# JiawangBian/SC-SfMLearner-Release

Measured on AMD Instinct MI355X. Metric: train images/sec (+ warp-loss ms/step) KITTI 256x832 RN18, higher is better.
Workload: dtype f32; 1 GPU; configs[1]: kitti 256x832, batch 12/GPU, 2 refs (seq 3), ResNet18 DispNet + ResNet18 PoseNet, ssim+mask+auto-mask, zeros padding, 1 scale; global_batch=12, parallelism=1 GPU, memory_format=contiguous (NCHW)

## Files before the change

__graft_entry__.py:

```python
import os
import sys

ROOT = os.path.dirname(os.path.abspath(__file__))
PKG = os.path.join(ROOT, "sc-sfmlearner-release_amd")
for p in (ROOT, PKG):
    if p not in sys.path:
        sys.path.insert(0, p)


def build() -> None:
    from scsfm_hip import _lib, build as hip_build
    path = hip_build.build(force=False)
    lib = _lib.CLib(path)
    assert lib._dll.scsfm_abi_version() == _lib.ABI_VERSION
    nets_path = hip_build.build_nets(force=False)
    nets = _lib.CLib(nets_path, _lib.NETS_HEADER, _lib.NETS_ABI_VERSION, "scsfm_nets_")
    eval_path = hip_build.build_eval(force=False)
    ev = _lib.CLib(eval_path, _lib.EVAL_HEADER, _lib.EVAL_ABI_VERSION, "scsfm_eval_")
    odom_path = hip_build.build_odom(force=False)
    od = _lib.CLib(odom_path, _lib.ODOM_HEADER, _lib.ODOM_ABI_VERSION, "scsfm_odom_")
    enc_path = hip_build.build_enc(force=False)
    enc = _lib.CLib(enc_path, _lib.ENC_HEADER, _lib.ENC_ABI_VERSION, "scsfm_enc_")
    import inverse_warp
    import loss_functions
    import models
    from scsfm_hip import decoder, depth_eval, encoder, odometry
    from oracle import scsfm_oracle
    print(f"[build] {path}: {len(lib.decls)} entry points resolved")
    print(f"[build] {nets_path}: {len(nets.decls)} entry points resolved")
    print(f"[build] {eval_path}: {len(ev.decls)} entry points resolved")
    print(f"[build] {odom_path}: {len(od.decls)} entry points resolved")
    print(f"[build] {enc_path}: {len(enc.decls)} entry points resolved")


def smoke() -> None:
    import torch

    import loss_functions as LF
    from oracle import scsfm_oracle as O
    from scsfm_hip import _lib, synth

    assert torch.cuda.is_available(), "smoke() needs a HIP device"
    lib = _lib.get()
    assert lib.path.endswith("libscsfm_hip.so")
    dev = torch.device("cuda:0")
    d = synth.make_batch(2, 128, 416, n_ref=2, seed=0, depth="smooth")

    def leaves(device):
        mv = lambda t: t.to(device).clone().requires_grad_(True)
        return ([mv(t) for t in d["tgt_depth"]], [[mv(t) for t in r] for r in d["ref_depths"]],
                [mv(p) for p in d["poses"]], [mv(p) for p in d["poses_inv"]])

    td, rd, ps, pi = leaves(dev)
    tgt, refs, K = d["tgt_img"].to(dev), [r.to(dev) for r in d["ref_imgs"]], d["intrinsics"].to(dev)
    photo, geom = LF.compute_photo_and_geometry_loss(tgt, refs, K, td, rd, ps, pi, 1, 1, 1, 1, "zeros")
    smooth = LF.compute_smooth_loss(td, tgt, rd, refs)
    (photo + 0.1 * smooth + 0.5 * geom).backward()
    torch.cuda.synchronize()

    td_c, rd_c, ps_c, pi_c = leaves("cpu")
    photo_c, geom_c = O.photo_and_geometry_loss(d["tgt_img"], d["ref_imgs"], d["intrinsics"], td_c, rd_c, ps_c, pi_c,
                                                1, 1, 1, 1, "zeros")
    smooth_c = O.smooth_loss(td_c, d["tgt_img"], rd_c, d["ref_imgs"])
    (photo_c + 0.1 * smooth_c + 0.5 * geom_c).backward()
    for name, a, b in (("photo", photo, photo_c), ("geom", geom, geom_c), ("smooth", smooth, smooth_c)):
        err = abs(float(a) - float(b))
        print(f"[smoke] {name}: hip {float(a):.7f} oracle {float(b):.7f} |d| {err:.2e}")
        assert err <= 1e-5, name
    pairs = [("g_tgt_depth", td[0].grad, td_c[0].grad), ("g_ref0_depth", rd[0][0].grad, rd_c[0][0].grad),
             ("g_ref1_depth", rd[1][0].grad, rd_c[1][0].grad), ("g_pose0", ps[0].grad, ps_c[0].grad),
             ("g_pose_inv1", pi[1].grad, pi_c[1].grad)]
    for name, a, b in pairs:
        scale = float(b.abs().max())
        bad = ((a.cpu() - b).abs() > 0.01 * scale).double().mean().item()
        print(f"[smoke] {name}: scale {scale:.3e} share of entries off by >1% of scale {bad:.2e}")
        assert bad <= 2e-3, name
    print("[smoke] ok")


if __name__ == "__main__":
    build()
    if "--smoke" in sys.argv:
        smoke()
```

sc-sfmlearner-release_amd/models/resnet_encoder.py:

```python
from __future__ import absolute_import, division, print_function

import numpy as np
import torch
import torch.nn as nn


_encoder_ops = None


def _E():
    global _encoder_ops
    if _encoder_ops is None:
        from scsfm_hip import encoder
        _encoder_ops = encoder
    return _encoder_ops


def _fused_applies(x, *bns):
    return x.is_cuda and _E().applies(x, *bns)


def _bn_act(x, bn, act, identity=None):
    if _fused_applies(x, bn) and (identity is None or _fused_applies(identity)):
        return _E().bn_act(x, bn, identity, relu=act is not None)
    out = bn(x)
    if identity is not None:
        out = out + identity
    return out if act is None else act(out)


def _downsample(ds, x):
    return _bn_act(ds[0](x), ds[1], None)


def _conv3x3(cin, cout, stride=1):
    return nn.Conv2d(cin, cout, kernel_size=3, stride=stride, padding=1, bias=False)


class BasicBlock(nn.Module):
    expansion = 1

    def __init__(self, inplanes, planes, stride=1, downsample=None):
        super().__init__()
        self.conv1 = _conv3x3(inplanes, planes, stride)
        self.bn1 = nn.BatchNorm2d(planes)
        self.relu = nn.ReLU(inplace=True)
        self.conv2 = _conv3x3(planes, planes)
        self.bn2 = nn.BatchNorm2d(planes)
        self.downsample = downsample

    def forward(self, x):
        identity = x if self.downsample is None else _downsample(self.downsample, x)
        out = _bn_act(self.conv1(x), self.bn1, self.relu)
        return _bn_act(self.conv2(out), self.bn2, self.relu, identity)

    def forward_reference(self, x):
        identity = x if self.downsample is None else self.downsample(x)
        out = self.relu(self.bn1(self.conv1(x)))
        out = self.bn2(self.conv2(out))
        return self.relu(out + identity)


class Bottleneck(nn.Module):
    expansion = 4

    def __init__(self, inplanes, planes, stride=1, downsample=None):
        super().__init__()
        self.conv1 = nn.Conv2d(inplanes, planes, kernel_size=1, bias=False)
        self.bn1 = nn.BatchNorm2d(planes)
        self.conv2 = _conv3x3(planes, planes, stride)
        self.bn2 = nn.BatchNorm2d(planes)
        self.conv3 = nn.Conv2d(planes, planes * 4, kernel_size=1, bias=False)
        self.bn3 = nn.BatchNorm2d(planes * 4)
        self.relu = nn.ReLU(inplace=True)
        self.downsample = downsample

    def forward(self, x):
        identity = x if self.downsample is None else _downsample(self.downsample, x)
        out = _bn_act(self.conv1(x), self.bn1, self.relu)
        out = _bn_act(self.conv2(out), self.bn2, self.relu)
        return _bn_act(self.conv3(out), self.bn3, self.relu, identity)

    def forward_reference(self, x):
        identity = x if self.downsample is None else self.downsample(x)
        out = self.relu(self.bn1(self.conv1(x)))
        out = self.relu(self.bn2(self.conv2(out)))
        out = self.bn3(self.conv3(out))
        return self.relu(out + identity)


class ResNet(nn.Module):

    def __init__(self, block, layers, num_classes=1000, num_input_images=1):
        super().__init__()
        self.inplanes = 64
        self.conv1 = nn.Conv2d(num_input_images * 3, 64, kernel_size=7, stride=2, padding=3, bias=False)
        self.bn1 = nn.BatchNorm2d(64)
        self.relu = nn.ReLU(inplace=True)
        self.maxpool = nn.MaxPool2d(kernel_size=3, stride=2, padding=1)
        self.layer1 = self._make_layer(block, 64, layers[0])
        self.layer2 = self._make_layer(block, 128, layers[1], stride=2)
        self.layer3 = self._make_layer(block, 256, layers[2], stride=2)
        self.layer4 = self._make_layer(block, 512, layers[3], stride=2)
        self.avgpool = nn.AdaptiveAvgPool2d((1, 1))
        self.fc = nn.Linear(512 * block.expansion, num_classes)
        for m in self.modules():
            if isinstance(m, nn.Conv2d):
                nn.init.kaiming_normal_(m.weight, mode='fan_out', nonlinearity='relu')
            elif isinstance(m, nn.BatchNorm2d):
                nn.init.constant_(m.weight, 1)
                nn.init.constant_(m.bias, 0)

    def _make_layer(self, block, planes, blocks, stride=1):
        downsample = None
        if stride != 1 or self.inplanes != planes * block.expansion:
            downsample = nn.Sequential(
                nn.Conv2d(self.inplanes, planes * block.expansion, kernel_size=1, stride=stride, bias=False),
                nn.BatchNorm2d(planes * block.expansion))
        layers = [block(self.inplanes, planes, stride, downsample)]
        self.inplanes = planes * block.expansion
        layers += [block(self.inplanes, planes) for _ in range(1, blocks)]
        return nn.Sequential(*layers)


_CFG = {18: (BasicBlock, [2, 2, 2, 2]), 50: (Bottleneck, [3, 4, 6, 3])}


def imagenet_weights_path(num_layers):
    import os
    root = os.environ.get("SCSFM_IMAGENET_WEIGHTS")
    if not root:
        return None
    path = os.path.join(root, "resnet{}.pth".format(num_layers))
    return path if os.path.exists(path) else None


class ResnetEncoder(nn.Module):

    def __init__(self, num_layers, pretrained, num_input_images=1):
        super().__init__()
        if num_layers not in _CFG:
            raise ValueError("{} is not a valid number of resnet layers".format(num_layers))
        block, layers = _CFG[num_layers]
        self.num_ch_enc = np.array([64, 64, 128, 256, 512])
        if num_layers > 34:
            self.num_ch_enc[1:] *= 4
        self.encoder = ResNet(block, layers, num_input_images=num_input_images)
        if pretrained:
            path = imagenet_weights_path(num_layers)
            if path is None:
                raise RuntimeError("ImageNet-pretrained weights are not reachable offline: set SCSFM_IMAGENET_WEIGHTS "
                                   "to a directory holding resnet{}.pth, or use --with-pretrain 0".format(num_layers))
            loaded = torch.load(path, map_location="cpu")
            loaded['conv1.weight'] = torch.cat([loaded['conv1.weight']] * num_input_images, 1) / num_input_images
            self.encoder.load_state_dict(loaded)
        for p in self.encoder.fc.parameters():
            p.requires_grad_(False)

    def forward(self, input_image):
        e = self.encoder
        f0 = _bn_act(e.conv1(input_image), e.bn1, e.relu)
        f1 = e.layer1(self._maxpool(f0))
        f2 = e.layer2(f1)
        f3 = e.layer3(f2)
        f4 = e.layer4(f3)
        self.features = [f0, f1, f2, f3, f4]
        return self.features

    def _maxpool(self, f0):
        e = self.encoder
        if f0.is_cuda and e.training and _E().pool_applies(f0):
            return _E().max_pool(f0)
        return e.maxpool(f0)

    def forward_reference(self, input_image):
        e = self.encoder
        f0 = e.relu(e.bn1(e.conv1(input_image)))
        feats, x = [f0], e.maxpool(f0)
        for layer in (e.layer1, e.layer2, e.layer3, e.layer4):
            for block in layer:
                x = block.forward_reference(x)
            feats.append(x)
        return feats
```

sc-sfmlearner-release_amd/scsfm_hip/_lib.py:

```python
from __future__ import annotations

import ctypes
import os
import re
import threading

import torch

HERE = os.path.dirname(os.path.abspath(__file__))
HEADER = os.path.join(os.path.dirname(os.path.dirname(HERE)), "include", "scsfm_hip.h")
LIB_PATH = os.environ.get("SCSFM_HIP_LIB") or os.path.join(HERE, "libscsfm_hip.so")

ABI_VERSION = 9

_CTYPES = {"int": ctypes.c_int, "unsigned": ctypes.c_uint, "size_t": ctypes.c_size_t, "double": ctypes.c_double}
_DECL = re.compile(r"^(int|size_t)\s+(scsfm_\w+)\s*\(([^)]*)\)\s*;", re.M | re.S)


def parse_header(path=HEADER):
    text = open(path).read()
    text = re.sub(r"/\*.*?\*/", "", text, flags=re.S)
    out = {}
    for ret, name, args in _DECL.findall(text):
        argtypes = []
        args = " ".join(args.split())
        if args and args != "void":
            for a in args.split(","):
                a = a.strip()
                if "*" in a:
                    argtypes.append(ctypes.c_void_p)
                else:
                    argtypes.append(_CTYPES[a.split()[0]])
        out[name] = (_CTYPES[ret], argtypes)
    return out


class ScsfmError(RuntimeError):
    pass


class CLib:

    def __init__(self, path, header=HEADER, abi=ABI_VERSION, prefix="scsfm_"):
        self.path = path
        self._dll = ctypes.CDLL(path)
        self.decls = parse_header(header)
        self._fn = {}
        self._prefix = prefix
        for name, (ret, argtypes) in self.decls.items():
            try:
                fn = getattr(self._dll, name)
            except AttributeError as e:
                raise ScsfmError(f"{path} does not export {name} (declared in {header})") from e
            fn.restype = ret
            fn.argtypes = argtypes
            self._fn[name] = fn
        if self._fn[prefix + "abi_version"]() != abi:
            raise ScsfmError(f"{path}: ABI version mismatch")

    def source_id(self):
        buf = ctypes.create_string_buffer(64)
        self._fn[self._prefix + "source_id"](buf, 64)
        return buf.value.decode()

    def call(self, name, *args):
        rc = self._fn[name](*args)
        if rc != 0:
            kind = "rejected argument" if rc == -1 else "hipError_t"
            raise ScsfmError(f"{name} failed with status {rc} ({kind})")

    def size(self, name, *args):
        return int(self._fn[name](*args))


_lock = threading.Lock()
_lib = None


def get() -> CLib:
    global _lib
    if _lib is None:
        with _lock:
            if _lib is None:
                from . import build as _build
                own = "SCSFM_HIP_LIB" not in os.environ
                if own and _build.is_stale():
                    have = _build.binary_source_id(LIB_PATH)
                    try:
                        _build.build()
                    except Exception as e:
                        what = f"was built from other sources ({have}) than the tree's ({_build.source_id()})" if have \
                            else "is missing (or carries no source id)"
                        raise ScsfmError(f"{LIB_PATH} {what} and cannot be built here: {e}") from e
                lib = CLib(LIB_PATH)
                if own and lib.source_id() != _build.source_id():
                    raise ScsfmError(f"{LIB_PATH}: its source id {lib.source_id()} is not the tree's {_build.source_id()}")
                _lib = lib
    return _lib


NETS_HEADER = os.path.join(os.path.dirname(os.path.dirname(HERE)), "include", "scsfm_nets.h")
NETS_LIB_PATH = os.path.join(HERE, "libscsfm_nets.so")
NETS_ABI_VERSION = 1
_nets = None


def get_nets() -> CLib:
    global _nets
    if _nets is None:
        with _lock:
            if _nets is None:
                from . import build as _build
                if _build.nets_is_stale():
                    have = _build.binary_source_id(NETS_LIB_PATH)
                    try:
                        _build.build_nets()
                    except Exception as e:
                        raise ScsfmError(f"{NETS_LIB_PATH} is stale or missing ({have}) and cannot be built here: {e}") \
                            from e
                lib = CLib(NETS_LIB_PATH, NETS_HEADER, NETS_ABI_VERSION, "scsfm_nets_")
                if lib.source_id() != _build.nets_source_id():
                    raise ScsfmError(f"{NETS_LIB_PATH}: its source id {lib.source_id()} is not the tree's "
                                     f"{_build.nets_source_id()}")
                _nets = lib
    return _nets


EVAL_HEADER = os.path.join(os.path.dirname(os.path.dirname(HERE)), "include", "scsfm_eval.h")
EVAL_LIB_PATH = os.path.join(HERE, "libscsfm_eval.so")
EVAL_ABI_VERSION = 1
_eval = None


def get_eval() -> CLib:
    global _eval
    if _eval is None:
        with _lock:
            if _eval is None:
                from . import build as _build
                if _build.eval_is_stale():
                    have = _build.binary_source_id(EVAL_LIB_PATH)
                    try:
                        _build.build_eval()
                    except Exception as e:
                        raise ScsfmError(f"{EVAL_LIB_PATH} is stale or missing ({have}) and cannot be built here: {e}") \
                            from e
                lib = CLib(EVAL_LIB_PATH, EVAL_HEADER, EVAL_ABI_VERSION, "scsfm_eval_")
                if lib.source_id() != _build.eval_source_id():
                    raise ScsfmError(f"{EVAL_LIB_PATH}: its source id {lib.source_id()} is not the tree's "
                                     f"{_build.eval_source_id()}")
                _eval = lib
    return _eval


ODOM_HEADER = os.path.join(os.path.dirname(os.path.dirname(HERE)), "include", "scsfm_odom.h")
ODOM_LIB_PATH = os.path.join(HERE, "libscsfm_odom.so")
ODOM_ABI_VERSION = 1
_odom = None


def get_odom() -> CLib:
    global _odom
    if _odom is None:
        with _lock:
            if _odom is None:
                from . import build as _build
                if _build.odom_is_stale():
                    have = _build.binary_source_id(ODOM_LIB_PATH)
                    try:
                        _build.build_odom()
                    except Exception as e:
                        raise ScsfmError(f"{ODOM_LIB_PATH} is stale or missing ({have}) and cannot be built here: {e}") \
                            from e
                lib = CLib(ODOM_LIB_PATH, ODOM_HEADER, ODOM_ABI_VERSION, "scsfm_odom_")
                if lib.source_id() != _build.odom_source_id():
                    raise ScsfmError(f"{ODOM_LIB_PATH}: its source id {lib.source_id()} is not the tree's "
                                     f"{_build.odom_source_id()}")
                _odom = lib
    return _odom


ENC_HEADER = os.path.join(os.path.dirname(os.path.dirname(HERE)), "include", "scsfm_enc.h")
ENC_LIB_PATH = os.path.join(HERE, "libscsfm_enc.so")
ENC_ABI_VERSION = 1
_enc = None


def get_enc() -> CLib:
    global _enc
    if _enc is None:
        with _lock:
            if _enc is None:
                from . import build as _build
                if _build.enc_is_stale():
                    have = _build.binary_source_id(ENC_LIB_PATH)
                    try:
                        _build.build_enc()
                    except Exception as e:
                        raise ScsfmError(f"{ENC_LIB_PATH} is stale or missing ({have}) and cannot be built here: {e}") \
                            from e
                lib = CLib(ENC_LIB_PATH, ENC_HEADER, ENC_ABI_VERSION, "scsfm_enc_")
                if lib.source_id() != _build.enc_source_id():
                    raise ScsfmError(f"{ENC_LIB_PATH}: its source id {lib.source_id()} is not the tree's "
                                     f"{_build.enc_source_id()}")
                _enc = lib
    return _enc
```

sc-sfmlearner-release_amd/scsfm_hip/build.py:

```python
from __future__ import annotations

import contextlib
import fcntl
import glob
import hashlib
import os
import shutil
import subprocess
import sys
import tempfile

HERE = os.path.dirname(os.path.abspath(__file__))
CSRC = os.path.join(os.path.dirname(HERE), "csrc")
LIB = os.path.join(HERE, "libscsfm_hip.so")
LOCK = LIB + ".lock"
LOG = LIB + ".buildlog"
INCLUDE = os.path.join(os.path.dirname(os.path.dirname(HERE)), "include")
NETS_CSRC = os.path.join(os.path.dirname(HERE), "csrc_nets")
NETS_LIB = os.path.join(HERE, "libscsfm_nets.so")
EVAL_CSRC = os.path.join(os.path.dirname(HERE), "csrc_eval")
EVAL_LIB = os.path.join(HERE, "libscsfm_eval.so")
ODOM_CSRC = os.path.join(os.path.dirname(HERE), "csrc_odom")
ODOM_LIB = os.path.join(HERE, "libscsfm_odom.so")
ENC_CSRC = os.path.join(os.path.dirname(HERE), "csrc_enc")
ENC_LIB = os.path.join(HERE, "libscsfm_enc.so")
ARCH = "gfx950"
FLAGS = ["-O3", "-std=c++17", "-fPIC", "-shared", f"--offload-arch={ARCH}", "-munsafe-fp-atomics",
         "-fno-gpu-rdc", "-Wall", "-Wno-unused-function",
         "-fno-slp-vectorize"]
ID_MARKER = b"scsfm-source-id:"


def sources():
    return sorted(glob.glob(os.path.join(CSRC, "*.hip")))


def deps():
    return sources() + sorted(glob.glob(os.path.join(CSRC, "*.h"))) + \
        [os.path.join(INCLUDE, "scsfm_hip.h")]


def nets_sources():
    return sorted(glob.glob(os.path.join(NETS_CSRC, "*.hip")))


def nets_deps():
    return nets_sources() + sorted(glob.glob(os.path.join(NETS_CSRC, "*.h"))) + [os.path.join(INCLUDE, "scsfm_nets.h")]


def eval_sources():
    return sorted(glob.glob(os.path.join(EVAL_CSRC, "*.hip")))


def eval_deps():
    return eval_sources() + sorted(glob.glob(os.path.join(EVAL_CSRC, "*.h"))) + [os.path.join(INCLUDE, "scsfm_eval.h")]


def odom_sources():
    return sorted(glob.glob(os.path.join(ODOM_CSRC, "*.hip")))


def odom_deps():
    return odom_sources() + sorted(glob.glob(os.path.join(ODOM_CSRC, "*.h"))) + [os.path.join(INCLUDE, "scsfm_odom.h")]


def enc_sources():
    return sorted(glob.glob(os.path.join(ENC_CSRC, "*.hip")))


def enc_deps():
    return enc_sources() + sorted(glob.glob(os.path.join(ENC_CSRC, "*.h"))) + [os.path.join(INCLUDE, "scsfm_enc.h")]


def _hash(files, extra=()):
    h = hashlib.sha256()
    for path in files:
        h.update(os.path.basename(path).encode())
        h.update(open(path, "rb").read())
    h.update(" ".join(FLAGS).encode())
    if extra:
        h.update(b"\0extra:" + " ".join(extra).encode())
    return h.hexdigest()[:16]


def source_id(extra=()):
    files = deps()
    if any("SCSFM_WITH_MARCH" in e or "variants" in e for e in extra):
        vsrc = os.path.join(os.path.dirname(os.path.dirname(HERE)), "variants", "src")
        files = files + sorted(p for p in glob.glob(os.path.join(vsrc, "*")) if os.path.isfile(p))
    return _hash(files, extra)


def nets_source_id():
    return _hash(nets_deps())


def eval_source_id():
    return _hash(eval_deps())


def odom_source_id():
    return _hash(odom_deps())


def enc_source_id():
    return _hash(enc_deps())


def binary_source_id(path=LIB):
    try:
        blob = open(path, "rb").read()
    except OSError:
        return None
    i = blob.find(ID_MARKER)
    if i < 0:
        return None
    j = i + len(ID_MARKER)
    return blob[j:j + 16].decode("ascii", "replace")


def is_stale():
    return binary_source_id(LIB) != source_id()


def nets_is_stale():
    return binary_source_id(NETS_LIB) != nets_source_id()


def eval_is_stale():
    return binary_source_id(EVAL_LIB) != eval_source_id()


def odom_is_stale():
    return binary_source_id(ODOM_LIB) != odom_source_id()


def enc_is_stale():
    return binary_source_id(ENC_LIB) != enc_source_id()


@contextlib.contextmanager
def _build_lock(lock=None):
    fd = os.open(lock or LOCK, os.O_CREAT | os.O_RDWR, 0o644)
    try:
        fcntl.flock(fd, fcntl.LOCK_EX)
        yield
    finally:
        try:
            fcntl.flock(fd, fcntl.LOCK_UN)
        finally:
            os.close(fd)


def build(force=False, verbose=True, extra=()):
    extra = tuple(extra)
    return _build(LIB, source_id(extra), sources(), extra, force, verbose)


def build_nets(force=False, verbose=True):
    return _build(NETS_LIB, nets_source_id(), nets_sources(), ("-I", INCLUDE), force, verbose)


def build_eval(force=False, verbose=True):
    return _build(EVAL_LIB, eval_source_id(), eval_sources(), ("-I", INCLUDE), force, verbose)


def build_odom(force=False, verbose=True):
    return _build(ODOM_LIB, odom_source_id(), odom_sources(), ("-I", INCLUDE), force, verbose)


def build_enc(force=False, verbose=True):
    return _build(ENC_LIB, enc_source_id(), enc_sources(), ("-I", INCLUDE), force, verbose)


def _build(lib, want, srcs, extra, force, verbose):
    if not force and binary_source_id(lib) == want:
        return lib
    with _build_lock(lib + ".lock"):
        if not force and binary_source_id(lib) == want:
            return lib
        hipcc = shutil.which("hipcc") or "/opt/rocm/bin/hipcc"
        name = os.path.basename(lib)
        if not os.path.exists(hipcc):
            raise RuntimeError(f"hipcc not found: {name} cannot be built on this machine")
        fd, tmp = tempfile.mkstemp(prefix=name[:-len(".so")] + ".", suffix=f".{os.getpid()}.tmp", dir=HERE)
        os.close(fd)
        try:
            cmd = [hipcc, *FLAGS, f'-DSCSFM_SOURCE_ID="{want}"', *extra, "-o", tmp, *srcs]
            if verbose:
                print("[scsfm_hip.build]", " ".join(cmd), flush=True)
            subprocess.run(cmd, check=True)
            os.chmod(tmp, 0o755)
            os.replace(tmp, lib)
            with open(lib + ".buildlog", "a") as f:
                f.write(f"{want} {os.getpid()}\n")
        finally:
            if os.path.exists(tmp):
                os.unlink(tmp)
    return lib


if __name__ == "__main__":
    build(force="--force" in sys.argv)
    build_nets(force="--force" in sys.argv)
    build_eval(force="--force" in sys.argv)
    build_odom(force="--force" in sys.argv)
    build_enc(force="--force" in sys.argv)
    print(LIB)
    print(NETS_LIB)
    print(EVAL_LIB)
    print(ODOM_LIB)
    print(ENC_LIB)
```

sc-sfmlearner-release_amd/scsfm_hip/encoder.py:

```python
from __future__ import annotations

import torch
from torch.autograd.function import once_differentiable

from . import _lib
from .capi import _stream


def _plain(t):
    return t.is_cuda and t.dtype == torch.float32 and t.is_contiguous()


def applies(x, *bns):
    if not (torch.is_tensor(x) and x.dim() == 4 and _plain(x) and x.numel() < 2 ** 31 and
            x.shape[0] * x.shape[2] * x.shape[3] >= 2):
        return False
    for bn in bns:
        if not (bn.training and bn.affine and bn.track_running_stats and bn.momentum is not None):
            return False
        if not all(_plain(t) for t in (bn.weight, bn.bias, bn.running_mean, bn.running_var)):
            return False
        if not (bn.num_batches_tracked.is_cuda and bn.num_batches_tracked.dtype == torch.int64):
            return False
    return True


def pool_applies(x):
    return torch.is_tensor(x) and x.dim() == 4 and _plain(x) and 0 < x.numel() < 2 ** 31


def _workspace(lib, x):
    B, C, H, W = x.shape
    n = lib.size("scsfm_enc_bn_workspace_bytes", B, C, H, W)
    return torch.empty(n // 8, dtype=torch.float64, device=x.device), n


class _BnAct(torch.autograd.Function):
    @staticmethod
    def forward(ctx, x, identity, weight, bias, bn, mode):
        lib = _lib.get_enc()
        B, C, H, W = x.shape
        if identity is not None and (identity.shape != x.shape or not _plain(identity)):
            raise ValueError(f"bn_act: identity {tuple(identity.shape)} does not match x {tuple(x.shape)}")
        y = torch.empty_like(x)
        stat = torch.empty((3, C), dtype=torch.float32, device=x.device)
        ws, n = _workspace(lib, x)
        lib.call("scsfm_enc_bn_fwd_f32", B, C, H, W, mode, float(bn.eps), float(bn.momentum), x.data_ptr(),
                 0 if identity is None else identity.data_ptr(), weight.data_ptr(), bias.data_ptr(), y.data_ptr(),
                 stat.data_ptr(), bn.running_mean.data_ptr(), bn.running_var.data_ptr(),
                 bn.num_batches_tracked.data_ptr(), ws.data_ptr(), n, _stream(x))
        ctx.mode = mode
        ctx.save_for_backward(x, weight, bias, stat, *((y,) if mode == 2 else ()))
        return y

    @staticmethod
    @once_differentiable
    def backward(ctx, g):
        lib = _lib.get_enc()
        g = g.contiguous()
        x, weight, bias, stat = ctx.saved_tensors[:4]
        y = ctx.saved_tensors[4] if ctx.mode == 2 else None
        B, C, H, W = x.shape
        dx = torch.empty_like(x)
        d_id = torch.empty_like(x) if ctx.mode == 2 else None
        dgamma = torch.empty(C, dtype=torch.float32, device=x.device)
        dbeta = torch.empty(C, dtype=torch.float32, device=x.device)
        ws, n = _workspace(lib, x)
        lib.call("scsfm_enc_bn_bwd_f32", B, C, H, W, ctx.mode, g.data_ptr(), x.data_ptr(),
                 0 if y is None else y.data_ptr(), weight.data_ptr(), bias.data_ptr(), stat.data_ptr(), dx.data_ptr(),
                 0 if d_id is None else d_id.data_ptr(), dgamma.data_ptr(), dbeta.data_ptr(), ws.data_ptr(), n,
                 _stream(x))
        return dx, d_id, dgamma, dbeta, None, None


class _MaxPool(torch.autograd.Function):
    @staticmethod
    def forward(ctx, x):
        B, C, H, W = x.shape
        PH, PW = (H - 1) // 2 + 1, (W - 1) // 2 + 1
        out = torch.empty((B, C, PH, PW), dtype=x.dtype, device=x.device)
        arg = torch.empty((B, C, PH, PW), dtype=torch.uint8, device=x.device)
        _lib.get_enc().call("scsfm_enc_maxpool_fwd_f32", B, C, H, W, x.data_ptr(), out.data_ptr(), arg.data_ptr(),
                            _stream(x))
        ctx.save_for_backward(arg)
        ctx.shape = (B, C, H, W)
        return out

    @staticmethod
    @once_differentiable
    def backward(ctx, g):
        g = g.contiguous()
        (arg,) = ctx.saved_tensors
        B, C, H, W = ctx.shape
        dx = torch.empty((B, C, H, W), dtype=g.dtype, device=g.device)
        _lib.get_enc().call("scsfm_enc_maxpool_bwd_f32", B, C, H, W, g.data_ptr(), arg.data_ptr(), dx.data_ptr(),
                            _stream(g))
        return dx


def bn_act(x, bn, identity=None, relu=True):
    if not applies(x, bn):
        raise ValueError("scsfm_hip.encoder.bn_act: CUDA fp32 contiguous NCHW input and a training-mode affine "
                         f"BatchNorm2d with running statistics only (got {x.device} {x.dtype} {tuple(x.shape)})")
    if identity is not None and not relu:
        raise ValueError("bn_act: the residual form ends in a ReLU")
    mode = 2 if identity is not None else (1 if relu else 0)
    return _BnAct.apply(x, identity, bn.weight, bn.bias, bn, mode)


def max_pool(x):
    if not pool_applies(x):
        raise ValueError("scsfm_hip.encoder.max_pool: CUDA fp32 contiguous NCHW tensors only "
                         f"(got {x.device} {x.dtype} {tuple(x.shape)})")
    return _MaxPool.apply(x)
```

Before: 137.1 images/s.

## Fuse encoder stem BatchNorm, ReLU and max-pool into one HIP kernel pair

Adds a new HIP library that computes the stem BatchNorm+ReLU output and the 3x3/stride-2 max-pool in the same pass, writing f0, the pooled tensor and argmax indices together. The backward kernel routes pooled gradients through the argmax, adds the skip gradient from f0, and computes the BN gradient in one sweep. The aim is to avoid re-reading the full-resolution f0 activation for the separate pool forward and to avoid materialising a separate pool-backward gradient. The trade-off is a more complex kernel with halo handling across strips and a new library to build and validate.

```diff
diff --git a/__graft_entry__.py b/__graft_entry__.py
--- a/__graft_entry__.py
+++ b/__graft_entry__.py
@@ -21,6 +21,8 @@
     od = _lib.CLib(odom_path, _lib.ODOM_HEADER, _lib.ODOM_ABI_VERSION, "scsfm_odom_")
     enc_path = hip_build.build_enc(force=False)
     enc = _lib.CLib(enc_path, _lib.ENC_HEADER, _lib.ENC_ABI_VERSION, "scsfm_enc_")
+    stem_path = hip_build.build_stem(force=False)
+    stem = _lib.CLib(stem_path, _lib.STEM_HEADER, _lib.STEM_ABI_VERSION, "scsfm_stem_")
     import inverse_warp
     import loss_functions
     import models
@@ -31,6 +33,7 @@
     print(f"[build] {eval_path}: {len(ev.decls)} entry points resolved")
     print(f"[build] {odom_path}: {len(od.decls)} entry points resolved")
     print(f"[build] {enc_path}: {len(enc.decls)} entry points resolved")
+    print(f"[build] {stem_path}: {len(stem.decls)} entry points resolved")
 
 
 def smoke() -> None:
@@ -75,6 +78,15 @@
         bad = ((a.cpu() - b).abs() > 0.01 * scale).double().mean().item()
         print(f"[smoke] {name}: scale {scale:.3e} share of entries off by >1% of scale {bad:.2e}")
         assert bad <= 2e-3, name
+    import torch.nn as nn
+    from scsfm_hip import encoder as E
+    assert _lib.get_stem().path.endswith("libscsfm_stem.so")
+    xs = torch.randn(2, 4, 6, 8, device=dev)
+    bn_a, bn_b = nn.BatchNorm2d(4).to(dev).train(), nn.BatchNorm2d(4).to(dev).train()
+    f0, pooled = E.bn_act(xs, bn_a, pool=True)
+    f0_ref = E.bn_act(xs, bn_b)
+    assert torch.equal(f0, f0_ref) and torch.equal(pooled, E.max_pool(f0_ref))
+    print("[smoke] stem: fused BatchNorm / ReLU / max-pool equals the separate ops")
     print("[smoke] ok")
 
 
diff --git a/include/scsfm_stem.h b/include/scsfm_stem.h
--- /dev/null
+++ b/include/scsfm_stem.h
@@ -0,0 +1,27 @@
+#ifndef SCSFM_STEM_H_
+#define SCSFM_STEM_H_
+
+#include <stddef.h>
+
+#ifdef __cplusplus
+extern "C" {
+#endif
+
+int scsfm_stem_abi_version(void);
+int scsfm_stem_source_id(char* buf, size_t n);
+
+size_t scsfm_stem_workspace_bytes(int B, int C, int H, int W);
+
+int scsfm_stem_fwd_f32(int B, int C, int H, int W, double eps, double momentum, const float* x, const float* gamma,
+                       const float* beta, float* f0, float* out, unsigned char* arg, float* stat, float* running_mean,
+                       float* running_var, long long* num_batches_tracked, void* ws, size_t ws_bytes, void* stream);
+
+int scsfm_stem_bwd_f32(int B, int C, int H, int W, const float* g_pool, const float* g_f0, const unsigned char* arg,
+                       const float* x, const float* gamma, const float* beta, const float* stat, float* dx,
+                       float* dgamma, float* dbeta, void* ws, size_t ws_bytes, void* stream);
+
+#ifdef __cplusplus
+}
+#endif
+
+#endif
diff --git a/sc-sfmlearner-release_amd/csrc_stem/scsfm_stem.hip b/sc-sfmlearner-release_amd/csrc_stem/scsfm_stem.hip
--- /dev/null
+++ b/sc-sfmlearner-release_amd/csrc_stem/scsfm_stem.hip
@@ -0,0 +1,599 @@
+#include <hip/hip_runtime.h>
+
+#include "scsfm_stem.h"
+
+namespace scsfm_stem {
+
+constexpr int kWave = 64;
+constexpr int kThreads = 256;
+constexpr int kWaves = kThreads / kWave;
+constexpr int kMaxSplit = 64;
+constexpr int kMaxPart = 256;
+constexpr int kTargetBlocks = 2048;
+constexpr int kUnroll = 4;
+
+template <int V>
+struct Pack {
+  float v[V];
+};
+template <int V>
+__device__ inline Pack<V> load(const float* __restrict__ p);
+template <>
+__device__ inline Pack<1> load<1>(const float* __restrict__ p) {
+  return {{p[0]}};
+}
+template <>
+__device__ inline Pack<4> load<4>(const float* __restrict__ p) {
+  const float4 t = *reinterpret_cast<const float4*>(p);
+  return {{t.x, t.y, t.z, t.w}};
+}
+
+__device__ inline int imin(int a, int b) { return a < b ? a : b; }
+__device__ inline int imax(int a, int b) { return a > b ? a : b; }
+
+struct Geo {
+  int C, HW, per, units;
+};
+template <int V>
+__device__ inline int offset_of(const Geo& g, int c, int u) {
+  const int b = u / g.per;
+  return (b * g.C + c) * g.HW + (u - b * g.per) * V;
+}
+__device__ inline void range(const Geo& g, int& u0, int& u1) {
+  const long long S = gridDim.y, s = blockIdx.y;
+  u0 = (int)(g.units * s / S);
+  u1 = (int)(g.units * (s + 1) / S);
+}
+
+__device__ inline double wave_sum(double v) {
+#pragma unroll
+  for (int d = kWave / 2; d > 0; d >>= 1) v += __shfl_down(v, d);
+  return v;
+}
+
+__device__ inline void block_sum_to(double a, double b, double* __restrict__ dst) {
+  __shared__ double red[2 * kWaves];
+  a = wave_sum(a);
+  b = wave_sum(b);
+  const int lane = threadIdx.x & (kWave - 1), wave = threadIdx.x >> 6;
+  if (lane == 0) {
+    red[2 * wave] = a;
+    red[2 * wave + 1] = b;
+  }
+  __syncthreads();
+  if (threadIdx.x == 0) {
+    double ta = red[0], tb = red[1];
+#pragma unroll
+    for (int w = 1; w < kWaves; ++w) {
+      ta += red[2 * w];
+      tb += red[2 * w + 1];
+    }
+    dst[0] = ta;
+    dst[1] = tb;
+  }
+}
+
+__device__ inline void stat_totals(const double* __restrict__ part, int c, int S, double& a, double& b) {
+  const int lane = threadIdx.x & (kWave - 1);
+  const double* src = part + 2 * ((size_t)c * S + imin(lane, S - 1));
+  a = wave_sum(lane < S ? src[0] : 0.0);
+  b = wave_sum(lane < S ? src[1] : 0.0);
+}
+
+__device__ inline void part_totals(const double* __restrict__ part, int c, int G, double& a, double& b) {
+  const int lane = threadIdx.x & (kWave - 1);
+  double sa = 0.0, sb = 0.0;
+  for (int j = lane; j < G; j += kWave) {
+    const double* src = part + 2 * ((size_t)c * G + j);
+    sa += src[0];
+    sb += src[1];
+  }
+  a = wave_sum(sa);
+  b = wave_sum(sb);
+}
+
+__device__ inline float relu(float v) { return v > 0.f ? v : (v != v ? v : 0.f); }
+__device__ inline float xhat_of(float x, float mean, float mean_lo, float invstd) { return ((x - mean) - mean_lo) * invstd; }
+__device__ inline float bn_value(float xh, float gamma, float beta) { return fmaf(xh, gamma, beta); }
+
+template <int V>
+__global__ __launch_bounds__(kThreads) void bn_stats_kernel(Geo geo, const float* __restrict__ x,
+                                                             double* __restrict__ part) {
+  const int c = blockIdx.x;
+  int u0, u1;
+  range(geo, u0, u1);
+  double s = 0.0, q = 0.0;
+  for (int u = u0 + (int)threadIdx.x; u < u1; u += kUnroll * kThreads) {
+    Pack<V> p[kUnroll];
+#pragma unroll
+    for (int j = 0; j < kUnroll; ++j) p[j] = load<V>(x + offset_of<V>(geo, c, imin(u + j * kThreads, u1 - 1)));
+#pragma unroll
+    for (int j = 0; j < kUnroll; ++j) {
+      if (u + j * kThreads < u1) {
+#pragma unroll
+        for (int k = 0; k < V; ++k) {
+          const double d = (double)p[j].v[k];
+          s += d;
+          q = fma(d, d, q);
+        }
+      }
+    }
+  }
+  block_sum_to(s, q, part + 2 * ((size_t)blockIdx.x * gridDim.y + blockIdx.y));
+}
+
+struct Plan {
+  int C, H, W, PH, PW, Wq, PB, NB, items;
+};
+struct Bn {
+  float mean, mean_lo, invstd, ga, be;
+};
+
+template <int V>
+__device__ inline void load_row(const float* __restrict__ row, int col0, int W, float (&v)[V]) {
+  if constexpr (V == 4) {
+    const float4 t = *reinterpret_cast<const float4*>(row + col0);
+    v[0] = t.x; v[1] = t.y; v[2] = t.z; v[3] = t.w;
+  } else {
+#pragma unroll
+    for (int j = 0; j < V; ++j) v[j] = col0 + j < W ? row[col0 + j] : 0.f;
+  }
+}
+template <int V>
+__device__ inline void store_row(float* __restrict__ row, int col0, int W, const float (&v)[V]) {
+  if constexpr (V == 4) {
+    float4 t;
+    t.x = v[0]; t.y = v[1]; t.z = v[2]; t.w = v[3];
+    *reinterpret_cast<float4*>(row + col0) = t;
+  } else {
+#pragma unroll
+    for (int j = 0; j < V; ++j)
+      if (col0 + j < W) row[col0 + j] = v[j];
+  }
+}
+
+__device__ inline float act(float x, const Bn& s) { return relu(bn_value(xhat_of(x, s.mean, s.mean_lo, s.invstd), s.ga, s.be)); }
+
+__device__ inline void take(float v, int at_v, float& best, int& at) {
+  if (v > best || v != v) {
+    best = v;
+    at = at_v;
+  }
+}
+__device__ inline void hfold(float a, bool va, float b, float c, bool vc, float& best, int& at) {
+  best = -INFINITY;
+  at = va ? 0 : 1;
+  if (va) take(a, 0, best, at);
+  take(b, 1, best, at);
+  if (vc) take(c, 2, best, at);
+}
+template <int V>
+__device__ inline void hfold_strip(const float (&y)[V], float l, int col0, int W, float (&best)[V / 2], int (&at)[V / 2]) {
+#pragma unroll
+  for (int q = 0; q < V / 2; ++q)
+    hfold(q == 0 ? l : y[imax(2 * q - 1, 0)], col0 + 2 * q > 0, y[2 * q], y[2 * q + 1], col0 + 2 * q + 1 < W, best[q],
+          at[q]);
+}
+
+template <int V>
+__global__ __launch_bounds__(kThreads) void stem_fwd_kernel(
+    Plan p, int S, int span, int rows, int segs, int groups, double inv_n, double unbias, double eps, double momentum,
+    const float* __restrict__ x, const float* __restrict__ gamma, const float* __restrict__ beta,
+    const double* __restrict__ part, float* __restrict__ f0, float* __restrict__ out, unsigned char* __restrict__ arg,
+    float* __restrict__ stat, float* __restrict__ running_mean, float* __restrict__ running_var,
+    long long* __restrict__ num_batches_tracked) {
+  constexpr int NP = V / 2;
+  __shared__ float sh[3];
+  __shared__ float edge[2][2][kThreads];
+  const int tid = threadIdx.x;
+  const int c = blockIdx.x / groups, grp = blockIdx.x - c * groups;
+  if (tid < kWave) {
+    double s, q;
+    stat_totals(part, c, S, s, q);
+    if (tid == 0) {
+      const double m = s * inv_n;
+      double var = q * inv_n - m * m;
+      if (var < 0.0) var = 0.0;
+      const float mf = (float)m, lo = (float)(m - (double)mf), is = (float)(1.0 / sqrt(var + eps));
+      sh[0] = mf;
+      sh[1] = is;
+      sh[2] = lo;
+      if (grp == 0) {
+        stat[c] = mf;
+        stat[p.C + c] = is;
+        stat[2 * p.C + c] = lo;
+        running_mean[c] = (float)((1.0 - momentum) * (double)running_mean[c] + momentum * m);
+        running_var[c] = (float)((1.0 - momentum) * (double)running_var[c] + momentum * var * unbias);
+        if (c == 0) num_batches_tracked[0] += 1;
+      }
+    }
+  }
+  __syncthreads();
+  const Bn bn = {sh[0], sh[2], sh[1], gamma[c], beta[c]};
+
+  const int ig = grp / segs, seg = grp - ig * segs;
+  const int r = tid / span, tl = tid - r * span;
+  const int strip = seg * kThreads + tl, item = ig * rows + r;
+  const bool live = r < rows && item < p.items && strip < p.Wq;
+  const int it = live ? item : 0, b = it / p.NB, ph0 = (it - b * p.NB) * p.PB;
+  const int col0 = live ? strip * V : 0, HW = p.H * p.W;
+  const size_t plane = (size_t)b * p.C + c;
+  const float* xp = x + plane * HW;
+  float* fp = f0 + plane * HW;
+  float* op = out + plane * p.PH * p.PW;
+  unsigned char* ap = arg + plane * p.PH * p.PW;
+  const bool recompute_left = live && tl == 0 && strip > 0;
+
+  float cb[NP];
+  int ca[NP];
+#pragma unroll
+  for (int q = 0; q < NP; ++q) {
+    cb[q] = -INFINITY;
+    ca[q] = 0;
+  }
+  int buf = 0;
+  {
+    const int h = 2 * ph0 - 1;
+    const bool on = live && h >= 0;
+    float y[V] = {};
+    if (on) {
+      load_row<V>(xp + h * p.W, col0, p.W, y);
+#pragma unroll
+      for (int j = 0; j < V; ++j) y[j] = act(y[j], bn);
+    }
+    edge[buf][0][tid] = y[V - 1];
+    __syncthreads();
+    if (on) {
+      float l = 0.f;
+      if (tl > 0) l = edge[buf][0][tid - 1];
+      else if (recompute_left) l = act(xp[h * p.W + col0 - 1], bn);
+      hfold_strip<V>(y, l, col0, p.W, cb, ca);
+    }
+    buf ^= 1;
+  }
+  for (int i = 0; i < p.PB; ++i) {
+    const int ph = ph0 + i, ha = 2 * ph, hb = ha + 1;
+    const bool on = live && ph < p.PH, onb = on && hb < p.H;
+    float ya[V] = {}, yb[V] = {};
+    if (on) load_row<V>(xp + ha * p.W, col0, p.W, ya);
+    if (onb) load_row<V>(xp + hb * p.W, col0, p.W, yb);
+    if (on) {
+#pragma unroll
+      for (int j = 0; j < V; ++j) ya[j] = act(ya[j], bn);
+      store_row<V>(fp + ha * p.W, col0, p.W, ya);
+    }
+    if (onb) {
+#pragma unroll
+      for (int j = 0; j < V; ++j) yb[j] = act(yb[j], bn);
+      store_row<V>(fp + hb * p.W, col0, p.W, yb);
+    }
+    edge[buf][0][tid] = ya[V - 1];
+    edge[buf][1][tid] = yb[V - 1];
+    __syncthreads();
+    if (on) {
+      float la = 0.f, lb = 0.f;
+      if (tl > 0) {
+        la = edge[buf][0][tid - 1];
+        lb = edge[buf][1][tid - 1];
+      } else if (recompute_left) {
+        la = act(xp[ha * p.W + col0 - 1], bn);
+        if (onb) lb = act(xp[hb * p.W + col0 - 1], bn);
+      }
+      float ab[NP], bb[NP];
+      int aa[NP], ba[NP];
+      hfold_strip<V>(ya, la, col0, p.W, ab, aa);
+      hfold_strip<V>(yb, lb, col0, p.W, bb, ba);
+      float best[NP];
+      int at[NP];
+#pragma unroll
+      for (int q = 0; q < NP; ++q) {
+        best[q] = -INFINITY;
+        at[q] = (ha > 0 ? 0 : 3) + (col0 + 2 * q > 0 ? 0 : 1);
+        if (ha > 0) take(cb[q], ca[q], best[q], at[q]);
+        take(ab[q], 3 + aa[q], best[q], at[q]);
+        if (onb) take(bb[q], 6 + ba[q], best[q], at[q]);
+        cb[q] = bb[q];
+        ca[q] = ba[q];
+      }
+      const int o = ph * p.PW + strip * NP;
+      if constexpr (V == 4) {
+        float2 t;
+        t.x = best[0]; t.y = best[1];
+        *reinterpret_cast<float2*>(op + o) = t;
+        *reinterpret_cast<unsigned short*>(ap + o) = (unsigned short)(at[0] | (at[1] << 8));
+      } else {
+        op[o] = best[0];
+        ap[o] = (unsigned char)at[0];
+      }
+    }
+    buf ^= 1;
+  }
+}
+
+template <int V>
+struct Pooled {
+  float g[V / 2 + 1];
+  int a[V / 2 + 1];
+};
+template <int V>
+__device__ inline Pooled<V> load_pooled(const float* __restrict__ gp, const unsigned char* __restrict__ ap, int ph,
+                                        int pw0, int PH, int PW) {
+  Pooled<V> r;
+#pragma unroll
+  for (int q = 0; q < V / 2 + 1; ++q) {
+    r.g[q] = 0.f;
+    r.a[q] = 255;
+  }
+  if (ph < PH) {
+    const int o = ph * PW + pw0;
+    if constexpr (V == 4) {
+      const float2 t = *reinterpret_cast<const float2*>(gp + o);
+      const unsigned s = *reinterpret_cast<const unsigned short*>(ap + o);
+      r.g[0] = t.x; r.g[1] = t.y;
+      r.a[0] = (int)(s & 255u); r.a[1] = (int)(s >> 8);
+      if (pw0 + 2 < PW) {
+        r.g[2] = gp[o + 2];
+        r.a[2] = ap[o + 2];
+      }
+    } else {
+#pragma unroll
+      for (int q = 0; q < 2; ++q)
+        if (pw0 + q < PW) {
+          r.g[q] = gp[o + q];
+          r.a[q] = ap[o + q];
+        }
+    }
+  }
+  return r;
+}
+template <int V>
+__device__ inline void route(const Pooled<V>& t, int base, float (&acc)[V]) {
+#pragma unroll
+  for (int j = 0; j < V; ++j) {
+    if (t.a[j / 2] == base + 1 + (j & 1)) acc[j] += t.g[j / 2];
+    if ((j & 1) && t.a[(j + 1) / 2] == base) acc[j] += t.g[(j + 1) / 2];
+  }
+}
+
+template <int V, bool SKIP, class F>
+__device__ inline void walk(const Plan& p, int c, int w0, int w1, const Bn& bn, const float* __restrict__ g_pool,
+                            const float* __restrict__ g_f0, const unsigned char* __restrict__ arg,
+                            const float* __restrict__ x, F&& f) {
+  const int HW = p.H * p.W;
+  for (int w = w0 + (int)threadIdx.x; w < w1; w += kThreads) {
+    const int item = w / p.Wq, strip = w - item * p.Wq, b = item / p.NB, ph0 = (item - b * p.NB) * p.PB;
+    const int ph1 = imin(p.PH, ph0 + p.PB), col0 = strip * V, pw0 = strip * (V / 2);
+    const size_t plane = (size_t)b * p.C + c;
+    const int base = (int)(plane * HW);
+    const float* gp = g_pool + plane * p.PH * p.PW;
+    const unsigned char* ap = arg + plane * p.PH * p.PW;
+    Pooled<V> top = load_pooled<V>(gp, ap, ph0, pw0, p.PH, p.PW);
+    for (int ph = ph0; ph < ph1; ++ph) {
+      const int oa = base + 2 * ph * p.W, ob = oa + p.W;
+      const bool onb = 2 * ph + 1 < p.H;
+      const Pooled<V> bot = load_pooled<V>(gp, ap, ph + 1, pw0, p.PH, p.PW);
+      float xa[V], xb[V] = {}, ta[V] = {}, tb[V] = {};
+      load_row<V>(x + oa, col0, p.W, xa);
+      if (onb) load_row<V>(x + ob, col0, p.W, xb);
+      if (SKIP) {
+        load_row<V>(g_f0 + oa, col0, p.W, ta);
+        if (onb) load_row<V>(g_f0 + ob, col0, p.W, tb);
+      }
+      float pa[V] = {}, pb[V] = {}, ma[V], mb[V], ha[V], hb[V];
+      route<V>(top, 3, pa);
+      route<V>(top, 6, pb);
+      route<V>(bot, 0, pb);
+#pragma unroll
+      for (int j = 0; j < V; ++j) {
+        ha[j] = xhat_of(xa[j], bn.mean, bn.mean_lo, bn.invstd);
+        hb[j] = xhat_of(xb[j], bn.mean, bn.mean_lo, bn.invstd);
+        const float ga = SKIP ? pa[j] + ta[j] : pa[j], gb = SKIP ? pb[j] + tb[j] : pb[j];
+        ma[j] = bn_value(ha[j], bn.ga, bn.be) <= 0.f ? 0.f : ga;
+        mb[j] = bn_value(hb[j], bn.ga, bn.be) <= 0.f ? 0.f : gb;
+      }
+      f(oa, col0, ma, ha);
+      if (onb) f(ob, col0, mb, hb);
+      top = bot;
+    }
+  }
+}
+
+__device__ inline void work_range(int work, int G, int g, int& w0, int& w1) {
+  w0 = (int)((long long)work * g / G);
+  w1 = (int)((long long)work * (g + 1) / G);
+}
+
+template <int V, bool SKIP>
+__global__ __launch_bounds__(kThreads) void stem_bwd_reduce_kernel(
+    Plan p, int G, const float* __restrict__ g_pool, const float* __restrict__ g_f0,
+    const unsigned char* __restrict__ arg, const float* __restrict__ x, const float* __restrict__ gamma,
+    const float* __restrict__ beta, const float* __restrict__ stat, double* __restrict__ part) {
+  const int c = blockIdx.x / G, g = blockIdx.x - c * G;
+  const Bn bn = {stat[c], stat[2 * p.C + c], stat[p.C + c], gamma[c], beta[c]};
+  int w0, w1;
+  work_range(p.items * p.Wq, G, g, w0, w1);
+  double sb = 0.0, sg = 0.0;
+  const int W = p.W;
+  walk<V, SKIP>(p, c, w0, w1, bn, g_pool, g_f0, arg, x, [&](int, int col0, const float (&m)[V], const float (&xh)[V]) {
+#pragma unroll
+    for (int j = 0; j < V; ++j)
+      if (V == 4 || col0 + j < W) {
+        const double gm = (double)m[j];
+        sb += gm;
+        sg = fma(gm, (double)xh[j], sg);
+      }
+  });
+  block_sum_to(sb, sg, part + 2 * (size_t)blockIdx.x);
+}
+
+template <int V, bool SKIP>
+__global__ __launch_bounds__(kThreads) void stem_bwd_dx_kernel(
+    Plan p, int G, double inv_n, const float* __restrict__ g_pool, const float* __restrict__ g_f0,
+    const unsigned char* __restrict__ arg, const float* __restrict__ x, const float* __restrict__ gamma,
+    const float* __restrict__ beta, const float* __restrict__ stat, const double* __restrict__ part,
+    float* __restrict__ dx, float* __restrict__ dgamma, float* __restrict__ dbeta) {
+  __shared__ float sh[2];
+  const int c = blockIdx.x / G, g = blockIdx.x - c * G;
+  if (threadIdx.x < kWave) {
+    double sb, sg;
+    part_totals(part, c, G, sb, sg);
+    if (threadIdx.x == 0) {
+      sh[0] = (float)(sb * inv_n);
+      sh[1] = (float)(sg * inv_n);
+      if (g == 0) {
+        dbeta[c] = (float)sb;
+        dgamma[c] = (float)sg;
+      }
+    }
+  }
+  __syncthreads();
+  const Bn bn = {stat[c], stat[2 * p.C + c], stat[p.C + c], gamma[c], beta[c]};
+  const float mb = sh[0], mg = sh[1], k1 = bn.ga * bn.invstd;
+  int w0, w1;
+  work_range(p.items * p.Wq, G, g, w0, w1);
+  const int W = p.W;
+  walk<V, SKIP>(p, c, w0, w1, bn, g_pool, g_f0, arg, x, [&](int off, int col0, const float (&m)[V], const float (&xh)[V]) {
+    float o[V];
+#pragma unroll
+    for (int j = 0; j < V; ++j) o[j] = ((m[j] - mb) - xh[j] * mg) * k1;
+    store_row<V>(dx + off, col0, W, o);
+  });
+}
+
+inline int ceil_div(long long a, long long b) { return (int)((a + b - 1) / b); }
+
+inline bool shape_ok(int B, int C, int H, int W) {
+  if (B <= 0 || C <= 0 || H <= 0 || W <= 0) return false;
+  const long long n = (long long)B * H * W;
+  return n >= 2 && n * C < (1ll << 31);
+}
+inline bool aligned(const void* p, size_t a) { return ((size_t)p & (a - 1)) == 0; }
+
+inline Geo geometry(int B, int C, int H, int W, bool vec) {
+  const int HW = H * W, per = vec ? HW / 4 : HW;
+  return {C, HW, per, B * per};
+}
+inline int splits(int C, int units) {
+  int S = ceil_div(kTargetBlocks, C);
+  const int most = ceil_div(units, kThreads);
+  if (S > most) S = most;
+  if (S > kMaxSplit) S = kMaxSplit;
+  return S < 1 ? 1 : S;
+}
+
+struct FwdGrid {
+  int span, rows, segs, groups;
+};
+inline FwdGrid fwd_grid(const Plan& p) {
+  FwdGrid f;
+  f.span = p.Wq < kThreads ? p.Wq : kThreads;
+  f.rows = kThreads / f.span;
+  f.segs = ceil_div(p.Wq, kThreads);
+  f.groups = ceil_div(p.items, f.rows) * f.segs;
+  return f;
+}
+inline int bwd_groups(const Plan& p) {
+  const int G = ceil_div((long long)p.items * p.Wq, kThreads);
+  return G > kMaxPart ? kMaxPart : G;
+}
+inline Plan plan(int B, int C, int H, int W, int V, bool forward) {
+  Plan p = {C, H, W, (H - 1) / 2 + 1, (W - 1) / 2 + 1, ceil_div(W, V), 1, 0, 0};
+  for (;; p.PB *= 2) {
+    p.NB = ceil_div(p.PH, p.PB);
+    p.items = B * p.NB;
+    const long long blocks = (long long)C * (forward ? fwd_grid(p).groups : bwd_groups(p));
+    if (blocks <= kTargetBlocks || p.PB >= p.PH) return p;
+  }
+}
+
+inline int launch_status() { return (int)hipGetLastError(); }
+
+}
+
+using namespace scsfm_stem;
+
+extern "C" {
+
+int scsfm_stem_abi_version(void) { return 1; }
+
+#ifndef SCSFM_SOURCE_ID
+#define SCSFM_SOURCE_ID "unknown"
+#endif
+static const char g_source_tag[] __attribute__((used)) = "scsfm-source-id:" SCSFM_SOURCE_ID;
+int scsfm_stem_source_id(char* buf, size_t n) {
+  const volatile char* id = g_source_tag + 16;
+  if (!buf || n == 0) return -1;
+  size_t i = 0;
+  for (; i + 1 < n && id[i]; ++i) buf[i] = id[i];
+  buf[i] = 0;
+  return 0;
+}
+
+size_t scsfm_stem_workspace_bytes(int B, int C, int H, int W) {
+  if (!shape_ok(B, C, H, W)) return 0;
+  return (size_t)C * kMaxPart * 2 * sizeof(double);
+}
+
+int scsfm_stem_fwd_f32(int B, int C, int H, int W, double eps, double momentum, const float* x, const float* gamma,
+                       const float* beta, float* f0, float* out, unsigned char* arg, float* stat, float* running_mean,
+                       float* running_var, long long* num_batches_tracked, void* ws, size_t ws_bytes, void* stream) {
+  if (!shape_ok(B, C, H, W) || !(eps >= 0.0) || !(momentum >= 0.0 && momentum <= 1.0) || !x || !gamma || !beta || !f0 ||
+      !out || !arg || !stat || !running_mean || !running_var || !num_batches_tracked || !ws || ((size_t)ws & 7) ||
+      ws_bytes < scsfm_stem_workspace_bytes(B, C, H, W))
+    return -1;
+  (void)hipGetLastError();
+  const double n = (double)B * H * W, inv_n = 1.0 / n, unbias = n / (n - 1.0);
+  double* part = (double*)ws;
+  const bool vec_stats = (H * W) % 4 == 0 && aligned(x, 16) && aligned(f0, 16);
+  const Geo geo = geometry(B, C, H, W, vec_stats);
+  const int S = splits(C, geo.units);
+  if (vec_stats) hipLaunchKernelGGL(bn_stats_kernel<4>, dim3(C, S), dim3(kThreads), 0, (hipStream_t)stream, geo, x, part);
+  else hipLaunchKernelGGL(bn_stats_kernel<1>, dim3(C, S), dim3(kThreads), 0, (hipStream_t)stream, geo, x, part);
+  const bool vec = W % 4 == 0 && aligned(x, 16) && aligned(f0, 16) && aligned(out, 8) && aligned(arg, 2);
+  const Plan p = plan(B, C, H, W, vec ? 4 : 2, true);
+  const FwdGrid f = fwd_grid(p);
+  const dim3 grid((unsigned)((long long)C * f.groups)), block(kThreads);
+  if (vec)
+    hipLaunchKernelGGL(stem_fwd_kernel<4>, grid, block, 0, (hipStream_t)stream, p, S, f.span, f.rows, f.segs, f.groups,
+                       inv_n, unbias, eps, momentum, x, gamma, beta, part, f0, out, arg, stat, running_mean, running_var,
+                       num_batches_tracked);
+  else
+    hipLaunchKernelGGL(stem_fwd_kernel<2>, grid, block, 0, (hipStream_t)stream, p, S, f.span, f.rows, f.segs, f.groups,
+                       inv_n, unbias, eps, momentum, x, gamma, beta, part, f0, out, arg, stat, running_mean, running_var,
+                       num_batches_tracked);
+  return launch_status();
+}
+
+#define SCSFM_STEM_BWD(V, SKIP)                                                                                          \
+  do {                                                                                                                   \
+    hipLaunchKernelGGL((stem_bwd_reduce_kernel<V, SKIP>), grid, block, 0, (hipStream_t)stream, p, G, g_pool, g_f0, arg,  \
+                       x, gamma, beta, stat, part);                                                                      \
+    hipLaunchKernelGGL((stem_bwd_dx_kernel<V, SKIP>), grid, block, 0, (hipStream_t)stream, p, G, inv_n, g_pool, g_f0,    \
+                       arg, x, gamma, beta, stat, part, dx, dgamma, dbeta);                                              \
+  } while (0)
+
+int scsfm_stem_bwd_f32(int B, int C, int H, int W, const float* g_pool, const float* g_f0, const unsigned char* arg,
+                       const float* x, const float* gamma, const float* beta, const float* stat, float* dx,
+                       float* dgamma, float* dbeta, void* ws, size_t ws_bytes, void* stream) {
+  if (!shape_ok(B, C, H, W) || !g_pool || !arg || !x || !gamma || !beta || !stat || !dx || !dgamma || !dbeta || !ws ||
+      ((size_t)ws & 7) || ws_bytes < scsfm_stem_workspace_bytes(B, C, H, W))
+    return -1;
+  (void)hipGetLastError();
+  const bool vec = W % 4 == 0 && aligned(x, 16) && aligned(dx, 16) && (!g_f0 || aligned(g_f0, 16)) &&
+                   aligned(g_pool, 8) && aligned(arg, 2);
+  const Plan p = plan(B, C, H, W, vec ? 4 : 2, false);
+  const int G = bwd_groups(p);
+  const dim3 grid((unsigned)((long long)C * G)), block(kThreads);
+  const double inv_n = 1.0 / ((double)B * H * W);
+  double* part = (double*)ws;
+  if (vec) {
+    if (g_f0) SCSFM_STEM_BWD(4, true);
+    else SCSFM_STEM_BWD(4, false);
+  } else {
+    if (g_f0) SCSFM_STEM_BWD(2, true);
+    else SCSFM_STEM_BWD(2, false);
+  }
+  return launch_status();
+}
+
+}
diff --git a/sc-sfmlearner-release_amd/models/resnet_encoder.py b/sc-sfmlearner-release_amd/models/resnet_encoder.py
--- a/sc-sfmlearner-release_amd/models/resnet_encoder.py
+++ b/sc-sfmlearner-release_amd/models/resnet_encoder.py
@@ -159,8 +159,13 @@
 
     def forward(self, input_image):
         e = self.encoder
-        f0 = _bn_act(e.conv1(input_image), e.bn1, e.relu)
-        f1 = e.layer1(self._maxpool(f0))
+        x = e.conv1(input_image)
+        if _fused_applies(x, e.bn1) and _E().pool_applies(x):
+            f0, pooled = _E().bn_act(x, e.bn1, relu=True, pool=True)
+        else:
+            f0 = _bn_act(x, e.bn1, e.relu)
+            pooled = self._maxpool(f0)
+        f1 = e.layer1(pooled)
         f2 = e.layer2(f1)
         f3 = e.layer3(f2)
         f4 = e.layer4(f3)
diff --git a/sc-sfmlearner-release_amd/scsfm_hip/_lib.py b/sc-sfmlearner-release_amd/scsfm_hip/_lib.py
--- a/sc-sfmlearner-release_amd/scsfm_hip/_lib.py
+++ b/sc-sfmlearner-release_amd/scsfm_hip/_lib.py
@@ -205,3 +205,30 @@
                                      f"{_build.enc_source_id()}")
                 _enc = lib
     return _enc
+
+
+STEM_HEADER = os.path.join(os.path.dirname(os.path.dirname(HERE)), "include", "scsfm_stem.h")
+STEM_LIB_PATH = os.path.join(HERE, "libscsfm_stem.so")
+STEM_ABI_VERSION = 1
+_stem = None
+
+
+def get_stem() -> CLib:
+    global _stem
+    if _stem is None:
+        with _lock:
+            if _stem is None:
+                from . import build as _build
+                if _build.stem_is_stale():
+                    have = _build.binary_source_id(STEM_LIB_PATH)
+                    try:
+                        _build.build_stem()
+                    except Exception as e:
+                        raise ScsfmError(f"{STEM_LIB_PATH} is stale or missing ({have}) and cannot be built here: {e}") \
+                            from e
+                lib = CLib(STEM_LIB_PATH, STEM_HEADER, STEM_ABI_VERSION, "scsfm_stem_")
+                if lib.source_id() != _build.stem_source_id():
+                    raise ScsfmError(f"{STEM_LIB_PATH}: its source id {lib.source_id()} is not the tree's "
+                                     f"{_build.stem_source_id()}")
+                _stem = lib
+    return _stem
diff --git a/sc-sfmlearner-release_amd/scsfm_hip/build.py b/sc-sfmlearner-release_amd/scsfm_hip/build.py
--- a/sc-sfmlearner-release_amd/scsfm_hip/build.py
+++ b/sc-sfmlearner-release_amd/scsfm_hip/build.py
@@ -24,6 +24,8 @@
 ODOM_LIB = os.path.join(HERE, "libscsfm_odom.so")
 ENC_CSRC = os.path.join(os.path.dirname(HERE), "csrc_enc")
 ENC_LIB = os.path.join(HERE, "libscsfm_enc.so")
+STEM_CSRC = os.path.join(os.path.dirname(HERE), "csrc_stem")
+STEM_LIB = os.path.join(HERE, "libscsfm_stem.so")
 ARCH = "gfx950"
 FLAGS = ["-O3", "-std=c++17", "-fPIC", "-shared", f"--offload-arch={ARCH}", "-munsafe-fp-atomics",
          "-fno-gpu-rdc", "-Wall", "-Wno-unused-function",
@@ -70,6 +72,14 @@
 
 def enc_deps():
     return enc_sources() + sorted(glob.glob(os.path.join(ENC_CSRC, "*.h"))) + [os.path.join(INCLUDE, "scsfm_enc.h")]
+
+
+def stem_sources():
+    return sorted(glob.glob(os.path.join(STEM_CSRC, "*.hip")))
+
+
+def stem_deps():
+    return stem_sources() + sorted(glob.glob(os.path.join(STEM_CSRC, "*.h"))) + [os.path.join(INCLUDE, "scsfm_stem.h")]
 
 
 def _hash(files, extra=()):
@@ -105,6 +115,10 @@
 
 def enc_source_id():
     return _hash(enc_deps())
+
+
+def stem_source_id():
+    return _hash(stem_deps())
 
 
 def binary_source_id(path=LIB):
@@ -137,6 +151,10 @@
 
 def enc_is_stale():
     return binary_source_id(ENC_LIB) != enc_source_id()
+
+
+def stem_is_stale():
+    return binary_source_id(STEM_LIB) != stem_source_id()
 
 
 @contextlib.contextmanager
@@ -171,6 +189,10 @@
 
 def build_enc(force=False, verbose=True):
     return _build(ENC_LIB, enc_source_id(), enc_sources(), ("-I", INCLUDE), force, verbose)
+
+
+def build_stem(force=False, verbose=True):
+    return _build(STEM_LIB, stem_source_id(), stem_sources(), ("-I", INCLUDE), force, verbose)
 
 
 def _build(lib, want, srcs, extra, force, verbose):
@@ -206,8 +228,10 @@
     build_eval(force="--force" in sys.argv)
     build_odom(force="--force" in sys.argv)
     build_enc(force="--force" in sys.argv)
+    build_stem(force="--force" in sys.argv)
     print(LIB)
     print(NETS_LIB)
     print(EVAL_LIB)
     print(ODOM_LIB)
     print(ENC_LIB)
+    print(STEM_LIB)
diff --git a/sc-sfmlearner-release_amd/scsfm_hip/encoder.py b/sc-sfmlearner-release_amd/scsfm_hip/encoder.py
--- a/sc-sfmlearner-release_amd/scsfm_hip/encoder.py
+++ b/sc-sfmlearner-release_amd/scsfm_hip/encoder.py
@@ -98,12 +98,66 @@
         return dx
 
 
-def bn_act(x, bn, identity=None, relu=True):
+class _BnReluPool(torch.autograd.Function):
+
+    @staticmethod
+    def forward(ctx, x, weight, bias, bn):
+        lib = _lib.get_stem()
+        B, C, H, W = x.shape
+        PH, PW = (H - 1) // 2 + 1, (W - 1) // 2 + 1
+        f0 = torch.empty_like(x)
+        out = torch.empty((B, C, PH, PW), dtype=x.dtype, device=x.device)
+        arg = torch.empty((B, C, PH, PW), dtype=torch.uint8, device=x.device)
+        stat = torch.empty((3, C), dtype=torch.float32, device=x.device)
+        n = lib.size("scsfm_stem_workspace_bytes", B, C, H, W)
+        ws = torch.empty(n // 8, dtype=torch.float64, device=x.device)
+        lib.call("scsfm_stem_fwd_f32", B, C, H, W, float(bn.eps), float(bn.momentum), x.data_ptr(), weight.data_ptr(),
+                 bias.data_ptr(), f0.data_ptr(), out.data_ptr(), arg.data_ptr(), stat.data_ptr(),
+                 bn.running_mean.data_ptr(), bn.running_var.data_ptr(), bn.num_batches_tracked.data_ptr(),
+                 ws.data_ptr(), n, _stream(x))
+        ctx.set_materialize_grads(False)
+        ctx.save_for_backward(x, weight, bias, stat, arg)
+        return f0, out
+
+    @staticmethod
+    @once_differentiable
+    def backward(ctx, g_f0, g_pool):
+        if g_f0 is None and g_pool is None:
+            return None, None, None, None
+        x, weight, bias, stat, arg = ctx.saved_tensors
+        B, C, H, W = x.shape
+        dx = torch.empty_like(x)
+        dgamma = torch.empty(C, dtype=torch.float32, device=x.device)
+        dbeta = torch.empty(C, dtype=torch.float32, device=x.device)
+        if g_f0 is not None:
+            g_f0 = g_f0.contiguous()
+        if g_pool is None:
+            lib = _lib.get_enc()
+            ws, n = _workspace(lib, x)
+            lib.call("scsfm_enc_bn_bwd_f32", B, C, H, W, 1, g_f0.data_ptr(), x.data_ptr(), 0, weight.data_ptr(),
+                     bias.data_ptr(), stat.data_ptr(), dx.data_ptr(), 0, dgamma.data_ptr(), dbeta.data_ptr(),
+                     ws.data_ptr(), n, _stream(x))
+            return dx, dgamma, dbeta, None
+        lib = _lib.get_stem()
+        g_pool = g_pool.contiguous()
+        n = lib.size("scsfm_stem_workspace_bytes", B, C, H, W)
+        ws = torch.empty(n // 8, dtype=torch.float64, device=x.device)
+        lib.call("scsfm_stem_bwd_f32", B, C, H, W, g_pool.data_ptr(), 0 if g_f0 is None else g_f0.data_ptr(),
+                 arg.data_ptr(), x.data_ptr(), weight.data_ptr(), bias.data_ptr(), stat.data_ptr(), dx.data_ptr(),
+                 dgamma.data_ptr(), dbeta.data_ptr(), ws.data_ptr(), n, _stream(x))
+        return dx, dgamma, dbeta, None
+
+
+def bn_act(x, bn, identity=None, relu=True, pool=False):
     if not applies(x, bn):
         raise ValueError("scsfm_hip.encoder.bn_act: CUDA fp32 contiguous NCHW input and a training-mode affine "
                          f"BatchNorm2d with running statistics only (got {x.device} {x.dtype} {tuple(x.shape)})")
     if identity is not None and not relu:
         raise ValueError("bn_act: the residual form ends in a ReLU")
+    if pool:
+        if identity is not None or not relu:
+            raise ValueError("bn_act: pool=True is relu(bn(x)) followed by the max-pool, without an identity")
+        return _BnReluPool.apply(x, bn.weight, bn.bias, bn)
     mode = 2 if identity is not None else (1 if relu else 0)
     return _BnAct.apply(x, identity, bn.weight, bn.bias, bn, mode)
 
```

New measurement: 140.7 images/s, median of 6. +2.7%, better.
